# praateekmahajan/moving-mnist-vae

Hardware: AMD Instinct MI355X
Metric: frames/sec/GPU VAE train step, 20×64×64 batch; ELBO vs CPU ref (higher is better)
Workload: dtype bf16; 1 GPU; BASELINE configs[1]: 256 clips x 20 frames x 64x64 per GPU per step (=5120 frames), conv-VAE z=128, Gaussian NLL sigma=0.1 + KL (normal_vae_1_kl_0_mmd), Adam, random-init weights, Bernoulli(0.0521) q=2 labels; parallelism=dp1, rccl_ranks=1, grad_exchange=none, bn=per-rank batch statistics

## Files before the change

include/mmvae.h:

```cpp
#ifndef MMVAE_H_
#define MMVAE_H_

#include <stddef.h>
#include <stdint.h>

#ifdef __cplusplus
extern "C" {
#endif

#if defined(__GNUC__)
#define MMVAE_API __attribute__((visibility("default")))
#else
#define MMVAE_API
#endif

#define MMVAE_OK 0
#define MMVAE_ERR_ARG (-1)
#define MMVAE_ERR_HIP (-2)
#define MMVAE_ERR_WORKSPACE (-3)
#define MMVAE_ERR_UNSUPPORTED (-4)

#define MMVAE_F32 0
#define MMVAE_BF16 1
#define MMVAE_FP8 2
// ... 23 lines not shown
                             void* workspace, size_t workspace_bytes, float* mu, float* logvar, int training, void* stream);
MMVAE_API int mmvae_encoder_bwd(mmvae_net* net, int N, const float* d_mu, const float* d_logvar, const float* params, float* grads,
                      void* workspace, size_t workspace_bytes, void* stream);
MMVAE_API int mmvae_decoder_fwd(mmvae_net* net, int N, const float* encoding, const float* params, float* bn_f32, int64_t* bn_i64,
                      void* workspace, size_t workspace_bytes, float* recon, int training, void* stream);
MMVAE_API int mmvae_decoder_bwd(mmvae_net* net, int N, const float* d_recon, const float* params, float* grads, void* workspace,
                      size_t workspace_bytes, float* d_encoding , void* stream);
MMVAE_API int mmvae_decoder_bwd_gauss(mmvae_net* net, int N, const float* target, float sigma, float coef, const float* gscale, const float* params,
                            float* grads, void* workspace, size_t workspace_bytes, float* d_enc, void* stream);

MMVAE_API int mmvae_net_defer_join(mmvae_net* net, int enable);
MMVAE_API int mmvae_net_join(mmvae_net* net, void* stream);
MMVAE_API void* mmvae_net_fork(mmvae_net* net, void* stream);
MMVAE_API void* mmvae_net_side_stream(mmvae_net* net);
MMVAE_API int mmvae_net_set_join_grad(mmvae_net* net, int enable);
MMVAE_API int mmvae_net_describe_routes(mmvae_net* net, int N, char* buf, int cap);

typedef int (*mmvae_allreduce_fn)(float* buf, int64_t n, void* stream, void* user);
MMVAE_API int mmvae_net_set_sync_bn(mmvae_net* net, mmvae_allreduce_fn fn, void* user, int world);

typedef struct mmvae_comm mmvae_comm;
#define MMVAE_COMM_ID_BYTES 128
MMVAE_API int mmvae_comm_unique_id(void* id_host );
MMVAE_API int mmvae_comm_init(mmvae_comm** out, int world, int rank, const void* id_host);
MMVAE_API int mmvae_comm_allreduce(mmvae_comm* comm, float* buf, int64_t n, void* stream);
MMVAE_API int mmvae_comm_destroy(mmvae_comm* comm);
MMVAE_API int mmvae_net_set_sync_bn_comm(mmvae_net* net, mmvae_comm* comm);
MMVAE_API int mmvae_net_set_sync_bn_comm2(mmvae_net* net, mmvae_comm* comm_main, mmvae_comm* comm_side);

MMVAE_API int mmvae_rsample_fwd(const float* mu, const float* logvar, const float* eps, float* enc, int64_t n, void* stream);
// ... 118 lines not shown
                       void* scratch, void* stream);
MMVAE_API int mmvae_conv2d_wgrad_pair(int dtype, const void* x, const void* dy, const void* dy_shortcut, float* dweight, float* dweight_sc, int N,
                            int H, int W, int Cin, int Cout, const float* pro_scale, const float* pro_shift, int pro_relu, void* scratch,
                            void* stream);
#define MMVAE_BN_SCRATCH_BYTES (16u << 20)
MMVAE_API int mmvae_batchnorm_fwd(int dtype, const void* y, int64_t npix, int C, const float* gamma, const float* beta, float* running_mean,
                        float* running_var, int64_t* nbt, float momentum, float eps, int relu, void* out, float* save_mean, float* save_istd,
                        void* scratch, void* stream);
MMVAE_API int mmvae_batchnorm_bwd(int dtype, const void* dout, const void* y, const void* out, int64_t npix, int C, const float* gamma,
                        const float* save_mean, const float* save_istd, void* dy, float* dgamma, float* dbeta, void* scratch, void* stream);
#define MMVAE_STEM_SCRATCH_BYTES 12800u
MMVAE_API int mmvae_stem_fwd(int dtype, const void* x, const float* weight, void* y, int N, int S, float* stats, void* scratch, void* stream);
MMVAE_API int mmvae_stem_bwd(int dtype, const void* g, const void* y0, const void* x, const float* weight, const float* gamma,
                   const float* bn_scale, const float* bn_shift, const float* save_mean, const float* save_istd, float* dweight,
                   float* dgamma, float* dbeta, int N, int S, void* scratch, void* stream);
MMVAE_API int mmvae_convT_bwd_fused(int dtype, const void* x, const void* dy, const float* weight, float* dweight, void* dx, int N, int H, int W,
                          int Cin, int Cout, int k, int stride, int pad, const float* pro_scale, const float* pro_shift, int pro_relu,
                          const void* x2, const float* w2, float* dw2, void* scratch, void* wscratch, void* stream);
MMVAE_API int mmvae_tail_join_fwd(int dtype, const void* y2, const float* s2, const float* b2, const void* ys, const float* ss, const float* bs,
                        const float* weight, const float* bias, float* r_raw, float* stats, int N, int H, int W, void* stream);
MMVAE_API int mmvae_tail_join_fwd_stream(int dtype, const void* y2, const float* s2, const float* b2, const void* ys, const float* ss, const float* bs,
                               const float* weight, const float* bias, float* r_raw, float* stats, int N, int H, int W, void* stream);
MMVAE_API int mmvae_tail_join_bwd_reduce(int dtype, const float* d_raw, const float* weight, int out_planes, const void* y2, const float* s2,
                               const float* b2, const void* ys, const float* ss, const float* bs, float* partials, float* wpartials,
                               int N, int H, int W, void* stream);
MMVAE_API int mmvae_tail_join_bwd_apply(int dtype, const float* d_raw, const float* weight, int out_planes, const void* y2, const float* s2,
                              const float* b2, const void* ys, const float* ss, const float* bs, const float* A2, const float* B2,
                              const float* C2, const float* As, const float* Bs, const float* Cs, void* dy2, void* dys, int N, int H, int W,
                              void* stream);
MMVAE_API int mmvae_upblock_bwd_fused(const float* d_raw, const float* tail_weight, const void* y2, const float* s2, const float* b2,
// ... 40 lines not shown
```

moving-mnist-vae_amd/_lib.py:

```python
from __future__ import annotations

import ctypes
import os
from ctypes import POINTER, c_char_p, c_double, c_float, c_int, c_int32, c_int64, c_size_t, c_uint64, c_void_p

import torch

_HERE = os.path.dirname(os.path.abspath(__file__))
LIB_PATH = os.environ.get("MMVAE_LIB_PATH") or os.path.join(_HERE, "libmmvae_hip.so")
_lib = None
ABI_VERSION = 3
SUM_PARTIALS = 1025
BN_SCRATCH_BYTES = 16 << 20
STEM_SCRATCH_BYTES = 12800

P = c_void_p

PROTOTYPES = {
    "mmvae_abi_version": (c_int, []),
    "mmvae_last_error": (c_char_p, []),
    "mmvae_net_create": (c_int, [POINTER(c_void_p), c_int, c_int, c_int, c_int, c_int, c_int]),
    "mmvae_net_create_ex": (c_int, [POINTER(c_void_p), c_int, c_int, c_int, c_int, c_int, c_int, c_int]),
    "mmvae_net_destroy": (None, [P]),
    "mmvae_net_sizes": (c_int, [P, POINTER(c_int64), POINTER(c_int64), POINTER(c_int32), POINTER(c_int64), POINTER(c_int32)]),
    "mmvae_net_num_entries": (c_int, [P]),
    "mmvae_net_entry": (c_int, [P, c_int, c_char_p, c_int, POINTER(c_int32), POINTER(c_int32), POINTER(c_int32), POINTER(c_int64)]),
    "mmvae_net_workspace_bytes": (c_size_t, [P, c_int]),
    "mmvae_encoder_fwd": (c_int, [P, c_int, P, P, P, P, P, c_size_t, P, P, c_int, P]),
    "mmvae_net_stage_labels": (c_int, [P, c_int, P, c_int, c_float, c_float, P, P, c_size_t, P]),
    "mmvae_encoder_fwd_staged": (c_int, [P, c_int, P, P, P, P, P, c_size_t, P, P, c_int, P]),
    "mmvae_encoder_bwd": (c_int, [P, c_int, P, P, P, P, P, c_size_t, P]),
    "mmvae_decoder_fwd": (c_int, [P, c_int, P, P, P, P, P, c_size_t, P, c_int, P]),
    "mmvae_decoder_bwd": (c_int, [P, c_int, P, P, P, P, c_size_t, P, P]),
    "mmvae_decoder_bwd_gauss": (c_int, [P, c_int, P, c_float, c_float, P, P, P, P, c_size_t, P, P]),
    "mmvae_net_defer_join": (c_int, [P, c_int]),
    "mmvae_net_join": (c_int, [P, P]),
    "mmvae_net_fork": (P, [P, P]),
    "mmvae_net_side_stream": (P, [P]),
    "mmvae_net_set_join_grad": (c_int, [P, c_int]),
    "mmvae_net_describe_routes": (c_int, [P, c_int, c_char_p, c_int]),
    "mmvae_net_set_sync_bn": (c_int, [P, P, P, c_int]),
    "mmvae_rsample_fwd": (c_int, [P, P, P, P, c_int64, P]),
    "mmvae_rsample_bwd": (c_int, [P, P, P, P, P, c_int64, P]),
    "mmvae_kl_fwd": (c_int, [P, P, c_int64, P, P]),
    "mmvae_kl_fwd_ex": (c_int, [P, P, c_int64, P, P, P]),
    "mmvae_kl_bwd": (c_int, [P, P, c_float, P, P, P, c_int64, P]),
    "mmvae_gauss_nll_fwd": (c_int, [P, P, c_int64, c_float, P, P]),
    "mmvae_gauss_nll_fwd_ex": (c_int, [P, P, c_int64, c_float, P, P, P]),
    "mmvae_gauss_nll_bwd": (c_int, [P, P, c_int64, c_float, c_float, P, P, P]),
    "mmvae_ce_fwd": (c_int, [P, P, P, c_int, c_int, c_int, P, P]),
    "mmvae_ce_fwd_ex": (c_int, [P, P, P, c_int, c_int, c_int, P, P, P]),
    "mmvae_ce_bwd": (c_int, [P, P, P, c_int, c_int, c_int, c_float, P, P, P]),
    "mmvae_mmd_fwd": (c_int, [P, P, c_int, c_int, P, P, P]),
    "mmvae_mmd_fwd_ex": (c_int, [P, P, c_int, c_int, P, P, P, P]),
# ... 32 lines not shown
    "mmvae_conv2d_dgrad_ex": (c_int, [c_int, c_int, P, P, P, c_int, c_int, c_int, c_int, c_int, c_int, c_int, c_int, c_int, P, P, c_int, P, P]),
    "mmvae_conv2d_wgrad": (c_int, [c_int, c_int, P, P, P, c_int, c_int, c_int, c_int, c_int, c_int, c_int, c_int, P, P, c_int, P, P]),
    "mmvae_conv2d_wgrad_pair": (c_int, [c_int, P, P, P, P, P, c_int, c_int, c_int, c_int, c_int, P, P, c_int, P, P]),
    "mmvae_rbf_kernel": (c_int, [P, P, c_int, c_int, c_int, P, P]),
    "mmvae_comm_unique_id": (c_int, [P]),
    "mmvae_comm_init": (c_int, [POINTER(c_void_p), c_int, c_int, P]),
    "mmvae_comm_allreduce": (c_int, [P, P, c_int64, P]),
    "mmvae_comm_destroy": (c_int, [P]),
    "mmvae_net_set_sync_bn_comm": (c_int, [P, P]),
    "mmvae_net_set_sync_bn_comm2": (c_int, [P, P, P]),
    "mmvae_convT_bwd_fused": (c_int, [c_int, P, P, P, P, P, c_int, c_int, c_int, c_int, c_int, c_int, c_int, c_int, P, P, c_int, P, P, P, P, P, P]),
    "mmvae_batchnorm_fwd": (c_int, [c_int, P, c_int64, c_int, P, P, P, P, P, c_float, c_float, c_int, P, P, P, P, P]),
    "mmvae_batchnorm_bwd": (c_int, [c_int, P, P, P, c_int64, c_int, P, P, P, P, P, P, P, P]),
    "mmvae_stem_fwd": (c_int, [c_int, P, P, P, c_int, c_int, P, P, P]),
    "mmvae_stem_bwd": (c_int, [c_int, P, P, P, P, P, P, P, P, P, P, P, P, c_int, c_int, P, P]),
    "mmvae_tail_join_fwd": (c_int, [c_int, P, P, P, P, P, P, P, P, P, P, c_int, c_int, c_int, P]),
    "mmvae_tail_join_fwd_stream": (c_int, [c_int, P, P, P, P, P, P, P, P, P, P, c_int, c_int, c_int, P]),
    "mmvae_tail_join_bwd_reduce": (c_int, [c_int, P, P, c_int, P, P, P, P, P, P, P, P, c_int, c_int, c_int, P]),
    "mmvae_tail_join_bwd_apply": (c_int, [c_int, P, P, c_int, P, P, P, P, P, P, P, P, P, P, P, P, P, P, c_int, c_int, c_int, P]),
    "mmvae_upblock_bwd_fused": (c_int, [P] * 27 + [c_int, P, P]),
    "mmvae_join_conv1x1_fwd": (c_int, [P, P, P, P, P, P, P, c_int, P, P, P, c_int64, P, P]),
    "mmvae_conv1x1_bwd_fused": (c_int, [P] * 13 + [c_int64, P, P]),
    "mmvae_upblock_tail_fwd": (c_int, [P] * 16 + [c_int, P, P]),
    "mmvae_upblock_tail_fwd_store": (c_int, [P] * 18 + [c_int, P, P]),
    "mmvae_convT4_stats": (c_int, [c_int, P, P, P, P, P, c_int, c_int, P, P]),
    "mmvae_pixelcnn_create": (c_int, [POINTER(c_void_p), c_int, c_int, c_int, c_int, c_int]),
    "mmvae_pixelcnn_destroy": (None, [P]),
    "mmvae_pixelcnn_num_params": (c_int64, [P]),
    "mmvae_pixelcnn_workspace_bytes": (c_size_t, [P, c_int, c_int]),
    "mmvae_pixelcnn_fwd": (c_int, [P, c_int, c_int, P, P, P, c_size_t, P, P]),
# ... 82 lines not shown
```

moving-mnist-vae_amd/csrc/capi.cpp:

```cpp
#include <cstring>
#include <new>

#include "../../include/mmvae.h"
#include "conv_ops.hpp"
#include "pixel_net.hpp"
#include "quantiser_fit.hpp"
#include "resample.hpp"
#include "vae_net.hpp"

namespace mmvae { const char* last_error(); }
using namespace mmvae;

struct mmvae_net { Net* net; };
struct mmvae_comm { Comm* c; };

static inline hipStream_t stream_of(void* s) { return static_cast<hipStream_t>(s); }

extern "C" {

int mmvae_abi_version(void) { return MMVAE_ABI_VERSION; }
const char* mmvae_last_error(void) { return last_error(); }

int mmvae_net_create(mmvae_net** out, int in_channels, int z, int out_channels, int image_size, int need_logvar, int dtype) {
  return mmvae_net_create_ex(out, in_channels, z, out_channels, image_size, need_logvar, dtype, 1);
// ... 89 lines not shown
  return MMVAE_OK;
}
int mmvae_net_join(mmvae_net* n, void* stream) {
  if (!n) { set_error("net_join: bad argument"); return MMVAE_ERR_ARG; }
  return n->net->join(stream_of(stream));
}

void* mmvae_net_fork(mmvae_net* n, void* stream) {
  if (!n) return stream;
  return reinterpret_cast<void*>(n->net->fork(stream_of(stream)));
}

int mmvae_net_set_join_grad(mmvae_net* n, int enable) {
  if (!n) { set_error("net_set_join_grad: bad argument"); return MMVAE_ERR_ARG; }
  n->net->set_join_grad(enable != 0);
  return MMVAE_OK;
}

int mmvae_net_describe_routes(mmvae_net* n, int N, char* buf, int cap) {
  if (!n || N <= 0 || cap < 0 || (!buf && cap > 0)) { set_error("net_describe_routes: bad argument"); return MMVAE_ERR_ARG; }
  std::string text;
  const int rc = n->net->describe_routes(N, text);
  if (rc < 0) return rc;
  if (cap > 0) { std::strncpy(buf, text.c_str(), cap - 1); buf[cap - 1] = 0; }
  return (int)text.size() + 1;
}

void* mmvae_net_side_stream(mmvae_net* n) { return n ? reinterpret_cast<void*>(n->net->side()) : nullptr; }

int mmvae_net_set_sync_bn(mmvae_net* n, mmvae_allreduce_fn fn, void* user, int world) {
// ... 446 lines not shown
                   void* scratch, void* st) {
  if (!scratch || N < 1) { set_error("stem_bwd: bad arguments"); return MMVAE_ERR_ARG; }
  if (!stem_bwd_fusable(Sz)) { set_error("stem_bwd: image size %d unsupported (64, 32, 16)", Sz); return MMVAE_ERR_UNSUPPORTED; }
  const int H1 = (Sz + 4 - 5) / 2 + 1;
  double* R = static_cast<double*>(scratch);
  float* gram = reinterpret_cast<float*>(R + 1024);
  const long gram_floats = 1024L * stem_bwd_part_floats();
  float* part = gram + gram_floats;
  const long part_floats = (long)(MMVAE_BN_SCRATCH_BYTES - 1024 * 8) / 4 - gram_floats;
  int rc = launch_stem_gram(dt, x, gram, gram_floats, R, N, Sz, H1, H1, stream_of(st));
  if (rc < 0) return rc;
  const int np = launch_stem_bwd(dt, g, y0, x, bn_scale, bn_shift, part, part_floats, N, Sz, H1, H1, stream_of(st));
  if (np < 0) return np;
  return launch_stem_bwd_finalize(part, np, R, w, nullptr, (double)N * H1 * H1, gamma, save_mean, save_istd, dgamma, dbeta, dw, stream_of(st));
}
int mmvae_tail_join_fwd(int dt, const void* y2, const float* s2, const float* b2, const void* ys, const float* ss, const float* bs,
                        const float* w, const float* bias, float* r_raw, float* stats, int N, int H, int W, void* st) {
  return launch_tail_join_fwd(dt, BnSide{y2, {s2, b2}}, BnSide{ys, {ss, bs}}, w, bias, r_raw, stats, N, H, W, stream_of(st));
}
int mmvae_tail_join_fwd_stream(int dt, const void* y2, const float* s2, const float* b2, const void* ys, const float* ss, const float* bs,
                               const float* w, const float* bias, float* r_raw, float* stats, int N, int H, int W, void* st) {
  return launch_tail_fwd_stream(dt, BnSide{y2, {s2, b2}}, BnSide{ys, {ss, bs}}, w, bias, r_raw, stats, N, H, W, stream_of(st));
}
int mmvae_tail_join_bwd_reduce(int dt, const float* d_raw, const float* w, int oc, const void* y2, const float* s2, const float* b2,
                               const void* ys, const float* ss, const float* bs, float* partials, float* wpartials, int N, int H, int W,
                               void* st) {
  return launch_tail_join_bwd_reduce(dt, d_raw, w, BnSide{y2, {s2, b2}}, BnSide{ys, {ss, bs}}, partials, oc, N, H, W, stream_of(st), wpartials);
}
int mmvae_tail_join_bwd_apply(int dt, const float* d_raw, const float* w, int oc, const void* y2, const float* s2, const float* b2,
                              const void* ys, const float* ss, const float* bs, const float* A2, const float* B2, const float* C2,
// ... 94 lines not shown
```

moving-mnist-vae_amd/csrc/conv_fstream.hip:

```cpp
#include <hip/hip_runtime.h>

#include <stdlib.h>
#include <string.h>

#include "kernels.hpp"
#include "tile_common.hpp"

namespace mmvae {

struct Conv3StreamArgs {
  const void* x; const void* w; const void* wsc; void* y; void* ysc;
  const float* pro_scale; const float* pro_shift; int pro_relu;
  float* stats; float* stats_sc;
  const void* ym; const float* ms; const float* mb;
  int N, Ho, Hi;
  int HS, nunits;
};

template <int S, bool SC, bool PRO, bool BS = false>
__global__ __launch_bounds__(256, 2) void conv3_stream_kernel(Conv3StreamArgs a) {
  static_assert(!BS || (S == 1 && !SC && !PRO), "backward sums: the stride-1 data gradient");
  constexpr int KS = 3, PAD = 1, WO = 16, WI = S * WO, CB = 64;
  constexpr int WL = WI + 2;
  constexpr int ROWB = WL * CB;
  constexpr int NSLOT = KS + S;
  constexpr int WAVE_LDS = NSLOT * ROWB;
  constexpr int RV = S * WI * CB / 1024;
  constexpr int NPRIME = (KS - S + S - 1) / S;
  extern __shared__ __attribute__((aligned(16))) char smem[];
  const int t = threadIdx.x, lane = t & 63, wv = __builtin_amdgcn_readfirstlane(t >> 6), gq = lane >> 4, r = lane & 15;
  char* ring = smem + 2048 + wv * WAVE_LDS;
  for (int s = 0; s < NSLOT; ++s) {
    if (lane < 4) *reinterpret_cast<Vec16*>(ring + s * ROWB + lane * 16) = Vec16{{0, 0, 0, 0}};
    else if (lane < 8) *reinterpret_cast<Vec16*>(ring + s * ROWB + (WL - 1) * CB + (lane - 4) * 16) = Vec16{{0, 0, 0, 0}};
  }
  Vec16 wA[KS * KS][2], wS[2];
#pragma unroll
  for (int m = 0; m < 2; ++m) {
    const int c = 8 * (r >> 2) + 4 * m + (r & 3);
#pragma unroll
    for (int tap = 0; tap < KS * KS; ++tap)
      wA[tap][m] = *reinterpret_cast<const Vec16*>(reinterpret_cast<const char*>(a.w) + ((c * KS * KS + tap) * 32 + 8 * gq) * 2);
    wS[m] = SC ? *reinterpret_cast<const Vec16*>(reinterpret_cast<const char*>(a.wsc) + (c * 32 + 8 * gq) * 2) : Vec16{{0, 0, 0, 0}};
  }
  float psc[8], psh[8];
  if (PRO) {
    const int c = (lane & 3) * 8;
#pragma unroll
    for (int j = 0; j < 8; ++j) { psc[j] = a.pro_scale[c + j]; psh[j] = a.pro_shift[c + j]; }
  }
  const float lo = a.pro_relu ? 0.f : -__builtin_inff();
  float bms[8], bmb[8];
  if (BS) {
#pragma unroll
    for (int j = 0; j < 8; ++j) { bms[j] = a.ms[8 * gq + j]; bmb[j] = a.mb[8 * gq + j]; }
  }
  Vec16 yv = Vec16{{0, 0, 0, 0}};
  float st[SC ? 4 : 2][8];
#pragma unroll
  for (int q = 0; q < (SC ? 4 : 2); ++q)
#pragma unroll
    for (int j = 0; j < 8; ++j) st[q][j] = 0.f;

  const bf16_t* __restrict__ X = reinterpret_cast<const bf16_t*>(a.x);
  const int nblk = gridDim.x;
  int u_first, u_step, u_end;
  if ((nblk & 7) == 0) {
    const int per = (a.nunits + 7) >> 3;
    const int lo_u = (blockIdx.x & 7) * per;
    u_first = lo_u + (blockIdx.x >> 3) * 4 + wv; u_step = (nblk >> 3) * 4; u_end = min(a.nunits, lo_u + per);
  } else { u_first = blockIdx.x * 4 + wv; u_step = nblk * 4; u_end = a.nunits; }
  const int nstrips = a.Ho / a.HS;
  const int nq = a.HS + NPRIME;

  Vec16 xv[RV];
  auto issue = [&](int u, int q) {
    const int n = u / nstrips, oh0 = (u - n * nstrips) * a.HS;
    const int top = S * (oh0 + q - NPRIME) + 1;
#pragma unroll
    for (int k = 0; k < RV; ++k) {
      const int byte = (lane + 64 * k) * 16;
      const int rr = byte / (WI * CB), off = byte - rr * (WI * CB);
      const int row = top - S + 1 + rr;
      xv[k] = Vec16{{0, 0, 0, 0}};
      if (row >= 0 && row < a.Hi) xv[k] = *reinterpret_cast<const Vec16*>(reinterpret_cast<const char*>(X) + (((long)n * a.Hi + row) * WI) * CB + off);
    }
    if (BS && q >= NPRIME)
      yv = *reinterpret_cast<const Vec16*>(reinterpret_cast<const char*>(a.ym) + ((((long)n * a.Ho + oh0 + q - NPRIME) * WO + r) * 32 + 8 * gq) * 2);
  };
  auto commit = [&](int u, int q) {
    const int n = u / nstrips, oh0 = (u - n * nstrips) * a.HS;
    const int top = S * (oh0 + q - NPRIME) + 1;
#pragma unroll
    for (int k = 0; k < RV; ++k) {
      const int byte = (lane + 64 * k) * 16;
      const int rr = byte / (WI * CB), off = byte - rr * (WI * CB);
      const int row = top - S + 1 + rr;
      Vec16 v = xv[k];
      if (PRO && row >= 0 && row < a.Hi) {
        float f[8];
        Elem<bf16_t>::unpack(v, f);
#pragma unroll
        for (int j = 0; j < 8; ++j) f[j] = fmaxf(f[j] * psc[j] + psh[j], lo);
        v = Elem<bf16_t>::pack(f);
      }
      *reinterpret_cast<Vec16*>(ring + ((row + 4 * NSLOT) % NSLOT) * ROWB + CB + off) = v;
    }
    (void)n;
  };

  int u = u_first, q = 0;
  if (u < u_end) issue(u, 0);
  while (u < u_end) {
    commit(u, q);
    const Vec16 ycur = yv;
    int un = u, qn = q + 1;
    if (qn == nq) { un = u + u_step; qn = 0; }
    if (un < u_end) issue(un, qn);
    __builtin_amdgcn_sched_barrier(0);
    if (q >= NPRIME) {
      const int n = u / nstrips, oh = (u - n * nstrips) * a.HS + q - NPRIME;
// ... 49 lines not shown
      if (r == 0) sb[wv * 128 + qq * 32 + 8 * gq + j] = v;
    }
  __syncthreads();
  if (t < (SC ? 128 : 64)) {
    const float v = (sb[t] + sb[128 + t]) + (sb[256 + t] + sb[384 + t]);
    float* dst = t < 64 ? a.stats : a.stats_sc;
    if (dst) dst[(long)blockIdx.x * 64 + (t & 63)] = v;
  }
}

bool conv3_stream_ok(int dt, int Cin, int Cout, int k, int s, int p, int Hin, int Win) {
  return dt == DT_BF16 && Cin == 32 && Cout == 32 && k == 3 && p == 1 && (s == 1 || s == 2) && Hin == Win && Win == 16 * s;
}

int launch_conv3_stream(int dt, int stride, const void* x, const void* w, const void* wsc, void* y, void* ysc, const float* pro_scale,
                        const float* pro_shift, int pro_relu, float* stats, float* stats_sc, int N, int Ho, hipStream_t s) {
  if (dt != DT_BF16 || (stride != 1 && stride != 2) || (wsc && stride != 2) || ((wsc != nullptr) != (ysc != nullptr))) {
    set_error("conv3_stream: bf16, stride 1 or 2, shortcut only with stride 2"); return MMVAE_ERR_UNSUPPORTED;
  }
  Conv3StreamArgs a; memset(&a, 0, sizeof(a));
  a.x = x; a.w = w; a.wsc = wsc; a.y = y; a.ysc = ysc; a.pro_scale = pro_scale; a.pro_shift = pro_shift; a.pro_relu = pro_relu;
  a.stats = stats; a.stats_sc = stats_sc; a.N = N; a.Ho = Ho; a.Hi = stride * Ho;
  a.HS = Ho % 8 == 0 ? 8 : Ho;
  a.nunits = N * (Ho / a.HS);
  int gx = stride == 1 ? 768 : 512;
  while (gx > 8 && (long)gx * 4 > a.nunits) gx -= 8;
  const bool pro = pro_scale != nullptr;
  const size_t lds = 2048 + 4 * (size_t)((3 + stride) * (stride * 16 + 2) * 64);
#define MMVAE_C3(S_, SC_, P_) hipLaunchKernelGGL((conv3_stream_kernel<S_, SC_, P_>), dim3(gx), dim3(256), lds, s, a)
  if (stride == 2) { if (wsc) { if (pro) MMVAE_C3(2, true, true); else MMVAE_C3(2, true, false); } else { if (pro) MMVAE_C3(2, false, true); else MMVAE_C3(2, false, false); } }
  else { if (pro) MMVAE_C3(1, false, true); else MMVAE_C3(1, false, false); }
#undef MMVAE_C3
  note_launch_bytes((double)N * 32 * 2.0 * ((double)a.Hi * a.Hi + (double)Ho * Ho * (wsc ? 2 : 1)));
  const int rc = check_launch("conv3_stream");
  return rc ? rc : gx;
}

int launch_conv3_stream_bwd(int dt, const void* dy, const void* w_flipped, void* dx, const void* ym, const float* ms, const float* mb, float* sums,
                            int N, int H, hipStream_t s) {
  if (dt != DT_BF16 || H != 16 || !ym || !ms || !mb || !sums) { set_error("conv3_stream_bwd: bf16, 16x16 maps, mask operand and sums required"); return MMVAE_ERR_UNSUPPORTED; }
  Conv3StreamArgs a; memset(&a, 0, sizeof(a));
  a.x = dy; a.w = w_flipped; a.y = dx; a.stats = sums; a.ym = ym; a.ms = ms; a.mb = mb; a.N = N; a.Ho = H; a.Hi = H;
  a.HS = 8; a.nunits = N * (H / a.HS);
  int gx = 768;
  while (gx > 8 && (long)gx * 4 > a.nunits) gx -= 8;
  const size_t lds = 2048 + 4 * (size_t)(4 * 18 * 64);
  hipLaunchKernelGGL((conv3_stream_kernel<1, false, false, true>), dim3(gx), dim3(256), lds, s, a);
  note_launch_bytes((double)N * 32 * 2.0 * 3.0 * H * H);
// ... 584 lines not shown
```

moving-mnist-vae_amd/csrc/kernels.hpp:

```cpp
#pragma once
#include "common.hpp"

namespace mmvae {

enum DType : int { DT_F32 = 0, DT_BF16 = 1 };
inline size_t dtype_size(int dt) { return dt == DT_F32 ? 4 : 2; }

struct Affine { const float* scale = nullptr; const float* shift = nullptr; };
struct BnCoef { const float* A = nullptr; const float* B = nullptr; const float* C = nullptr; };
struct BnSide { const void* y = nullptr; Affine fwd; BnCoef bwd; };

struct Tap { int dh, dw; };
constexpr int kMaxTaps = 25;
constexpr int kMaxPhases = 4;
struct Phase { int ph, pw, Hq, Wq, ntaps, tap0; long w_off;  };
struct GatherArgs {
  const void* x; const void* w; void* y;
  const float* pro_scale; const float* pro_shift; int pro_relu;
  const float* bias;
  float* stats;
  int accumulate;
  int N, Hi, Wi, Cin, Ho, Wo, Cout;
  int SI, SO;
  int nphase; Phase phases[kMaxPhases]; Tap taps[kMaxTaps];
// ... 132 lines not shown
  int cols_valid, K_valid;
  int fp8;
  int frag;
};
int launch_pack(int dt, const PackArgs& a, hipStream_t s);
void pack_batch_begin();
int pack_batch_flush(int dt, hipStream_t s);

int launch_stem_im2col(int dt, const void* x, void* col, int N, int H, int W, int Ho, int Wo, hipStream_t s);

bool stem_bwd_fusable(int S);
bool conv3_stream_ok(int dt, int Cin, int Cout, int k, int s, int p, int Hin, int Win);
int launch_conv3_stream_bwd(int dt, const void* dy, const void* w_flipped, void* dx, const void* ym, const float* ms, const float* mb, float* sums,
                            int N, int H, hipStream_t s);
int launch_conv3_stream(int dt, int stride, const void* x, const void* w, const void* wsc, void* y, void* ysc, const float* pro_scale,
                        const float* pro_shift, int pro_relu, float* stats, float* stats_sc, int N, int Ho, hipStream_t s);
bool convT4_stream_ok(int dt, int Cin, int Cout, int k, int s, int p, int Hin, int Win);
int launch_convT4_stream(int dt, const void* x, const void* w_up, void* y, const float* pro_scale, const float* pro_shift, int pro_relu, float* stats,
                         int N, int Hin, hipStream_t s, int f8out = 0);
bool tail_fwd_stream_ok(int dt, int OC, int H, int W);
int launch_tail_fwd_stream(int dt, const BnSide& y2, const BnSide& ys, const float* w, const float* bias, float* r_raw, float* stats, int N, int H,
                           int W, hipStream_t s, int f8in = 0);
bool up5_tail_fwd_ok(int dt, int OC, int C, int Cin, int Hin, int Hout);
int launch_up5_tail_fwd(const BnSide& y1, const void* w2_up, const BnSide& xin, const void* wu_up, Affine bn2, Affine bns, const float* w,
                        const float* bias, float* r_raw, float* stats, int N, hipStream_t s, void* y2 = nullptr, void* ys = nullptr);
bool stem_fwd_stream_ok(int dt, int S);
int launch_stem_fwd_stream(int dt, const void* x, const float* w, void* y, float* stats, int N, int S, hipStream_t s);
int stem_bwd_part_floats();
int launch_stem_gram(int dt, const void* x, float* scratch, long scratch_cap_floats, double* R, int N, int S, int Ho, int Wo, hipStream_t s);
int launch_stem_bwd(int dt, const void* g, const void* y0, const void* x, const float* ms, const float* mb, float* partials,
                    long partials_cap_floats, int N, int S, int Ho, int Wo, hipStream_t s);
// ... 135 lines not shown
```

moving-mnist-vae_amd/csrc/vae_net.cpp:

```cpp
#include "vae_net.hpp"

#include <algorithm>
#include <cmath>
#include <cstdlib>
#include <cstring>

#include "conv_ops.hpp"

namespace mmvae {

#define MM_TRY(expr)            \
  do {                          \
    int rc__ = (expr);          \
    if (rc__ < 0) return rc__;  \
  } while (0)

static inline long align_up(long v, long a) { return (v + a - 1) / a * a; }
static inline int down_size(int H, int k, int s, int p) { return conv_down_size(H, k, s, p); }

void Net::add_entry(const std::string& name, std::initializer_list<int> shape, int kind, long off) {
  Entry e; e.name = name; e.ndim = (int)shape.size(); e.kind = kind; e.offset = off;
  int i = 0; for (int d : shape) e.shape[i++] = d;
  for (; i < 4; ++i) e.shape[i] = 1;
  entries.push_back(e);
// ... 583 lines not shown
    np = launch_gather_gemm(dt(), dt(), a, s);
  }
  MM_TRY(np);
  MM_TRY(bn_fwd(ps, bn0, np, (double)N * H1 * W1, s));
  const void* xin = base + P.y0;
  const float* xs = ps.rows(bn0).scale;
  const float* xb = ps.rows(bn0).shift;
  if (cfg.blocks > 1) MM_TRY(fill_consts(ps, s));
  for (size_t i = 0; i < enc.size(); ++i) {
    Block& B = enc[i];
    const double cnt = (double)N * B.Hout * B.Wout;
    const BnRows r1 = ps.rows(B.b1);
    const BnSide s2 = ps.rows(B.b2).side(base + B.y2), sc = ps.shortcut(B, xin);
    const bool stream1 = B.r.fwd_c1_cs_stream, stream2 = B.r.fwd_c2_stream, fork = !B.identity && !stream1;
    if (stream1) {
      np = launch_conv3_stream(dt(), 2, xin, ps.packed(B.c1.packD), ps.packed(B.cs.packD), base + B.y1,
                               base + B.ys, xs, xb, 1, stats, stats ? stats + kPartialFloats : nullptr, N, B.Hout, s);
      MM_TRY(np);
      MM_TRY(bn_fwd(ps, B.bs, np, cnt, s, kPartialFloats, B.cs.wscale));
      MM_TRY(bn_fwd(ps, B.b1, np, cnt, s, 0, B.c1.wscale));
    } else if (!B.identity) {
      if (fork) MM_TRY(side_fork(s));
      hipStream_t ss = fork ? wgrad_stream(s) : s;
      np = run_down(ps, B.cs, xin, B.Hin, B.Win, base + B.ys, B.Hout, B.Wout, xs, xb, 1, stats ? stats + kPartialFloats : nullptr, 0, dt(), ss);
      MM_TRY(np);
      MM_TRY(bn_fwd(ps, B.bs, np, cnt, ss, kPartialFloats, B.cs.wscale));
    }
    if (!stream1) {
      np = run_down(ps, B.c1, xin, B.Hin, B.Win, base + B.y1, B.Hout, B.Wout, xs, xb, 1, stats, 0, dt(), s);
      MM_TRY(np);
      MM_TRY(bn_fwd(ps, B.b1, np, cnt, s, 0, B.c1.wscale));
    }
// ... 397 lines not shown
```

moving-mnist-vae_amd/csrc/vae_net.hpp:

```cpp
#pragma once
#include <string>
#include <vector>

#include "comm.hpp"
#include "conv_ops.hpp"
#include "kernels.hpp"

namespace mmvae {

struct NetCfg { int in_ch, z, out_ch, S, need_logvar, dtype, blocks, fp8; };

enum EntryKind : int { EK_PARAM = 0, EK_BN_F32 = 1, EK_BN_I64 = 2 };
struct Entry { std::string name; int ndim; int shape[4]; int kind; long offset; };

struct ConvW { long off; int D0, D1, k, s, p; long packD, packU; int Hl = 0;  bool tr = false;  bool fp8 = false; float wscale = 1.f;
               bool fragD = false, fragU = false;  };
struct Bn {
  long g_off, b_off, rm_off, rv_off; int nbt_idx; int C; long ws;
  enum Row { MEAN, ISTD, SCALE, SHIFT, COEF_A, COEF_B, COEF_C, kRows };
  long row_floats() const { return (C + 3L) / 4 * 4; }
  long row(Row r) const { return ws + r * row_floats(); }
  long scratch_floats() const { return kRows * row_floats(); }
};
struct BnRows {
// ... 132 lines not shown
               const ConvW* w2 = nullptr, const void* x2 = nullptr);
  int run_up(const Pass& ps, const ConvW& w, const void* S, int Hs, int Ws, void* L, int Hl, int Wl,
             const float* pro_s, const float* pro_b, int relu, float* stats, int accumulate, hipStream_t s,
             const ConvW* w2 = nullptr, const void* x2 = nullptr);
  int run_wgrad(const Pass& ps, const ConvW& w, const void* P, int Hs, int Ws, const float* proP_s, const float* proP_b,
                const void* G, int Hl, int Wl, const float* proG_s, const float* proG_b, hipStream_t s);
  int reduce_wgrad_parts(const Pass& ps, const ConvW& w, const float* parts, int nparts, int ntaps, hipStream_t s);
  bool defer_join_ = false;
  int (*ar_fn_)(float*, long long, void*, void*) = nullptr; void* ar_user_ = nullptr; int ar_world_ = 1;
  Comm* comm_ = nullptr; Comm* comm_side_ = nullptr;
  int sync_rows(const Pass& ps, const float* partials, int nparts, int width, hipStream_t s, float** out, int row_stride = 0);
 public:
  void set_defer_join(bool v) { defer_join_ = v; }
  bool join_grad_ = true;
  void set_join_grad(bool v) { join_grad_ = v; plan_.N = -1; }
  typedef int (*AllReduceFn)(float* buf, long long n, void* stream, void* user);
  void set_sync_bn(AllReduceFn fn, void* user, int world) { ar_fn_ = fn; ar_user_ = user; ar_world_ = fn ? world : 1; comm_ = comm_side_ = nullptr; }
  void set_sync_bn_comm(Comm* c, Comm* side = nullptr) { comm_ = c; comm_side_ = c ? side : nullptr; ar_fn_ = nullptr; ar_user_ = nullptr; ar_world_ = c ? comm_world(c) : 1; }
  bool sync_bn_on() const { return ar_fn_ != nullptr || comm_ != nullptr; }
  int join(hipStream_t s) { return side_join(s); }
  hipStream_t side() const { return side_state_ == 1 ? side_ : nullptr; }
  hipStream_t fork(hipStream_t s) { return side_fork(s) == MMVAE_OK ? wgrad_stream(s) : s; }
 private:
  int bn_fwd(const Pass& ps, const Bn& bn, int nparts, double count, hipStream_t s, long part_off = 0, float in_scale = 1.f);
  int fold_bn_eval(const Pass& ps, int which, hipStream_t s);
  long l1c2_flip = 0; bool eval_folded_ = false;
  bool store8 = false;
  int fill_consts(const Pass& ps, hipStream_t s);
  int bn_backward_coefs(const Pass& ps, const Bn& bn, int nparts, int ny, int which, double count, hipStream_t s, float* dbias_conv = nullptr);
  BnBwdFinalizeArgs bwd_finalize_args(const Pass& ps, const Bn& bn, const float* partials, int nparts, int ny, int which, double count) const;
// ... 8 lines not shown
```

Before: 867,300 frames/s.

## Recompute stem conv output inside encoder layer1 kernel from the raw image

In training with a 64x64 input, the encoder layer1 stride-2 conv kernel now reads the raw bf16 image. It recomputes the stem's 5x5 conv output on the fly with MFMA, then applies BN+ReLU before the 3x3 conv and shortcut. This avoids reading the 32-channel stem activation back from global memory. The cost is extra LDS for an image patch ring, redundant stem arithmetic per tile, and a second rounding path that must match the stored stem output used in backward.

Result: no change. 870,000 frames/s, median of 5 (+0.3%).

```diff
diff --git a/include/mmvae.h b/include/mmvae.h
--- a/include/mmvae.h
+++ b/include/mmvae.h
@@ -61,6 +61,7 @@
 MMVAE_API void* mmvae_net_fork(mmvae_net* net, void* stream);
 MMVAE_API void* mmvae_net_side_stream(mmvae_net* net);
 MMVAE_API int mmvae_net_set_join_grad(mmvae_net* net, int enable);
+MMVAE_API int mmvae_net_set_stem_recompute(mmvae_net* net, int enable);
 MMVAE_API int mmvae_net_describe_routes(mmvae_net* net, int N, char* buf, int cap);
 
 typedef int (*mmvae_allreduce_fn)(float* buf, int64_t n, void* stream, void* user);
@@ -209,6 +210,8 @@
 MMVAE_API int mmvae_stem_bwd(int dtype, const void* g, const void* y0, const void* x, const float* weight, const float* gamma,
                    const float* bn_scale, const float* bn_shift, const float* save_mean, const float* save_istd, float* dweight,
                    float* dgamma, float* dbeta, int N, int S, void* scratch, void* stream);
+MMVAE_API int mmvae_stem_block1_fwd(int dtype, const void* x, const float* weight, const float* bn_scale, const float* bn_shift, const float* w1,
+                          const float* ws, void* y1, void* ys, float* stats1, float* stats_s, int N, int S, void* scratch, void* stream);
 MMVAE_API int mmvae_convT_bwd_fused(int dtype, const void* x, const void* dy, const float* weight, float* dweight, void* dx, int N, int H, int W,
                           int Cin, int Cout, int k, int stride, int pad, const float* pro_scale, const float* pro_shift, int pro_relu,
                           const void* x2, const float* w2, float* dw2, void* scratch, void* wscratch, void* stream);
diff --git a/moving-mnist-vae_amd/_lib.py b/moving-mnist-vae_amd/_lib.py
--- a/moving-mnist-vae_amd/_lib.py
+++ b/moving-mnist-vae_amd/_lib.py
@@ -38,6 +38,7 @@
     "mmvae_net_fork": (P, [P, P]),
     "mmvae_net_side_stream": (P, [P]),
     "mmvae_net_set_join_grad": (c_int, [P, c_int]),
+    "mmvae_net_set_stem_recompute": (c_int, [P, c_int]),
     "mmvae_net_describe_routes": (c_int, [P, c_int, c_char_p, c_int]),
     "mmvae_net_set_sync_bn": (c_int, [P, P, P, c_int]),
     "mmvae_rsample_fwd": (c_int, [P, P, P, P, c_int64, P]),
@@ -100,6 +101,7 @@
     "mmvae_batchnorm_bwd": (c_int, [c_int, P, P, P, c_int64, c_int, P, P, P, P, P, P, P, P]),
     "mmvae_stem_fwd": (c_int, [c_int, P, P, P, c_int, c_int, P, P, P]),
     "mmvae_stem_bwd": (c_int, [c_int, P, P, P, P, P, P, P, P, P, P, P, P, c_int, c_int, P, P]),
+    "mmvae_stem_block1_fwd": (c_int, [c_int] + [P] * 10 + [c_int, c_int, P, P]),
     "mmvae_tail_join_fwd": (c_int, [c_int, P, P, P, P, P, P, P, P, P, P, c_int, c_int, c_int, P]),
     "mmvae_tail_join_fwd_stream": (c_int, [c_int, P, P, P, P, P, P, P, P, P, P, c_int, c_int, c_int, P]),
     "mmvae_tail_join_bwd_reduce": (c_int, [c_int, P, P, c_int, P, P, P, P, P, P, P, P, c_int, c_int, c_int, P]),
diff --git a/moving-mnist-vae_amd/csrc/capi.cpp b/moving-mnist-vae_amd/csrc/capi.cpp
--- a/moving-mnist-vae_amd/csrc/capi.cpp
+++ b/moving-mnist-vae_amd/csrc/capi.cpp
@@ -127,6 +127,12 @@
 int mmvae_net_set_join_grad(mmvae_net* n, int enable) {
   if (!n) { set_error("net_set_join_grad: bad argument"); return MMVAE_ERR_ARG; }
   n->net->set_join_grad(enable != 0);
+  return MMVAE_OK;
+}
+
+int mmvae_net_set_stem_recompute(mmvae_net* n, int enable) {
+  if (!n) { set_error("net_set_stem_recompute: bad argument"); return MMVAE_ERR_ARG; }
+  n->net->set_stem_recompute(enable != 0);
   return MMVAE_OK;
 }
 
@@ -603,6 +609,16 @@
   if (np < 0) return np;
   return launch_stem_bwd_finalize(part, np, R, w, nullptr, (double)N * H1 * H1, gamma, save_mean, save_istd, dgamma, dbeta, dw, stream_of(st));
 }
+int mmvae_stem_block1_fwd(int dt, const void* x, const float* w, const float* bn_scale, const float* bn_shift, const float* w1, const float* ws,
+                          void* y1, void* ys, float* stats1, float* stats_s, int N, int Sz, void* scratch, void* st) {
+  if (!scratch || !x || !w || !bn_scale || !bn_shift || !w1 || !ws || !y1 || !ys || N < 1) { set_error("stem_block1_fwd: bad arguments"); return MMVAE_ERR_ARG; }
+  if (dt != DT_BF16 || Sz != 64 || !stem_fwd_stream_ok(dt, Sz)) { set_error("stem_block1_fwd: bf16 and 64 x 64 images only"); return MMVAE_ERR_UNSUPPORTED; }
+  char* p1 = static_cast<char*>(scratch);
+  char* ps = p1 + 32 * 32 * 9 * 2;
+  int rc = op_pack_down(dt, geom_for(0, 32, 32, 3, 2, 1), w1, p1, stream_of(st)); if (rc < 0) return rc;
+  rc = op_pack_down(dt, geom_for(0, 32, 32, 1, 2, 0), ws, ps, stream_of(st)); if (rc < 0) return rc;
+  return launch_conv3_stream(dt, 2, nullptr, p1, ps, y1, ys, bn_scale, bn_shift, 1, stats1, stats_s, N, 16, stream_of(st), x, w);
+}
 int mmvae_tail_join_fwd(int dt, const void* y2, const float* s2, const float* b2, const void* ys, const float* ss, const float* bs,
                         const float* w, const float* bias, float* r_raw, float* stats, int N, int H, int W, void* st) {
   return launch_tail_join_fwd(dt, BnSide{y2, {s2, b2}}, BnSide{ys, {ss, bs}}, w, bias, r_raw, stats, N, H, W, stream_of(st));
diff --git a/moving-mnist-vae_amd/csrc/conv_fstream.hip b/moving-mnist-vae_amd/csrc/conv_fstream.hip
--- a/moving-mnist-vae_amd/csrc/conv_fstream.hip
+++ b/moving-mnist-vae_amd/csrc/conv_fstream.hip
@@ -13,18 +13,22 @@
   const float* pro_scale; const float* pro_shift; int pro_relu;
   float* stats; float* stats_sc;
   const void* ym; const float* ms; const float* mb;
+  const void* img; const float* w0;
   int N, Ho, Hi;
   int HS, nunits;
 };
 
-template <int S, bool SC, bool PRO, bool BS = false>
+constexpr int kImgPw = 72, kImgSlots = 8;
+
+template <int S, bool SC, bool PRO, bool BS = false, bool IMG = false>
 __global__ __launch_bounds__(256, 2) void conv3_stream_kernel(Conv3StreamArgs a) {
   static_assert(!BS || (S == 1 && !SC && !PRO), "backward sums: the stride-1 data gradient");
+  static_assert(!IMG || (S == 2 && PRO && !BS), "input rows from the image: the stride-2 conv behind the stem's BatchNorm + ReLU");
   constexpr int KS = 3, PAD = 1, WO = 16, WI = S * WO, CB = 64;
   constexpr int WL = WI + 2;
   constexpr int ROWB = WL * CB;
   constexpr int NSLOT = KS + S;
-  constexpr int WAVE_LDS = NSLOT * ROWB;
+  constexpr int WAVE_LDS = NSLOT * ROWB + (IMG ? kImgSlots * kImgPw * 4 : 0);
   constexpr int RV = S * WI * CB / 1024;
   constexpr int NPRIME = (KS - S + S - 1) / S;
   extern __shared__ __attribute__((aligned(16))) char smem[];
@@ -43,9 +47,26 @@
       wA[tap][m] = *reinterpret_cast<const Vec16*>(reinterpret_cast<const char*>(a.w) + ((c * KS * KS + tap) * 32 + 8 * gq) * 2);
     wS[m] = SC ? *reinterpret_cast<const Vec16*>(reinterpret_cast<const char*>(a.wsc) + (c * 32 + 8 * gq) * 2) : Vec16{{0, 0, 0, 0}};
   }
+  float* const patch = reinterpret_cast<float*>(ring + NSLOT * ROWB);
+  Vec16 wA0[2];
+  int toff[8];
+  const bool tap_in = gq < 3;
+  if constexpr (IMG) {
+    for (int i = lane; i < kImgSlots * kImgPw; i += 64) patch[i] = 0.f;
+#pragma unroll
+    for (int m = 0; m < 2; ++m) {
+      const int c = 8 * (r >> 2) + 4 * m + (r & 3);
+      float f[8];
+#pragma unroll
+      for (int j = 0; j < 8; ++j) { const int tap = 8 * gq + j; f[j] = tap < 25 ? a.w0[c * 25 + tap] : 0.f; }
+      wA0[m] = Elem<bf16_t>::pack(f);
+    }
+#pragma unroll
+    for (int j = 0; j < 8; ++j) { const int tap = 8 * gq + j; toff[j] = tap < 25 ? (tap / 5) * kImgPw + tap % 5 + 2 * r + 2 : 0; }
+  }
   float psc[8], psh[8];
   if (PRO) {
-    const int c = (lane & 3) * 8;
+    const int c = (IMG ? gq : (lane & 3)) * 8;
 #pragma unroll
     for (int j = 0; j < 8; ++j) { psc[j] = a.pro_scale[c + j]; psh[j] = a.pro_shift[c + j]; }
   }
@@ -73,38 +94,86 @@
   const int nstrips = a.Ho / a.HS;
   const int nq = a.HS + NPRIME;
 
-  Vec16 xv[RV];
+  Vec16 xv[IMG ? 1 : RV];
+  const int irow = lane >> 3, icol = (lane & 7) * 8;
   auto issue = [&](int u, int q) {
     const int n = u / nstrips, oh0 = (u - n * nstrips) * a.HS;
     const int top = S * (oh0 + q - NPRIME) + 1;
-#pragma unroll
-    for (int k = 0; k < RV; ++k) {
-      const int byte = (lane + 64 * k) * 16;
-      const int rr = byte / (WI * CB), off = byte - rr * (WI * CB);
-      const int row = top - S + 1 + rr;
-      xv[k] = Vec16{{0, 0, 0, 0}};
-      if (row >= 0 && row < a.Hi) xv[k] = *reinterpret_cast<const Vec16*>(reinterpret_cast<const char*>(X) + (((long)n * a.Hi + row) * WI) * CB + off);
-    }
-    if (BS && q >= NPRIME)
-      yv = *reinterpret_cast<const Vec16*>(reinterpret_cast<const char*>(a.ym) + ((((long)n * a.Ho + oh0 + q - NPRIME) * WO + r) * 32 + 8 * gq) * 2);
+    if constexpr (IMG) {
+      const int row = 2 * (top - 1) - 2 + irow;
+      xv[0] = Vec16{{0, 0, 0, 0}};
+      if (irow < 7 && (q == 0 || irow >= 3) && row >= 0 && row < 2 * a.Hi)
+        xv[0] = *reinterpret_cast<const Vec16*>(reinterpret_cast<const bf16_t*>(a.img) + (((long)n * 2 * a.Hi + row) * (2 * WI) + icol));
+    } else {
+#pragma unroll
+      for (int k = 0; k < RV; ++k) {
+        const int byte = (lane + 64 * k) * 16;
+        const int rr = byte / (WI * CB), off = byte - rr * (WI * CB);
+        const int row = top - S + 1 + rr;
+        xv[k] = Vec16{{0, 0, 0, 0}};
+        if (row >= 0 && row < a.Hi) xv[k] = *reinterpret_cast<const Vec16*>(reinterpret_cast<const char*>(X) + (((long)n * a.Hi + row) * WI) * CB + off);
+      }
+      if (BS && q >= NPRIME)
+        yv = *reinterpret_cast<const Vec16*>(reinterpret_cast<const char*>(a.ym) + ((((long)n * a.Ho + oh0 + q - NPRIME) * WO + r) * 32 + 8 * gq) * 2);
+    }
   };
   auto commit = [&](int u, int q) {
     const int n = u / nstrips, oh0 = (u - n * nstrips) * a.HS;
     const int top = S * (oh0 + q - NPRIME) + 1;
-#pragma unroll
-    for (int k = 0; k < RV; ++k) {
-      const int byte = (lane + 64 * k) * 16;
-      const int rr = byte / (WI * CB), off = byte - rr * (WI * CB);
-      const int row = top - S + 1 + rr;
-      Vec16 v = xv[k];
-      if (PRO && row >= 0 && row < a.Hi) {
+    if constexpr (IMG) {
+      const int rb = 2 * (top - 1) - 2;
+      if (irow < 7 && (q == 0 || irow >= 3)) {
         float f[8];
-        Elem<bf16_t>::unpack(v, f);
-#pragma unroll
-        for (int j = 0; j < 8; ++j) f[j] = fmaxf(f[j] * psc[j] + psh[j], lo);
-        v = Elem<bf16_t>::pack(f);
-      }
-      *reinterpret_cast<Vec16*>(ring + ((row + 4 * NSLOT) % NSLOT) * ROWB + CB + off) = v;
+        Elem<bf16_t>::unpack(xv[0], f);
+        float* d = patch + ((rb + irow) & (kImgSlots - 1)) * kImgPw + 4 + icol;
+        *reinterpret_cast<float4*>(d) = make_float4(f[0], f[1], f[2], f[3]);
+        *reinterpret_cast<float4*>(d + 4) = make_float4(f[4], f[5], f[6], f[7]);
+      }
+#pragma unroll
+      for (int e = 0; e < 2; ++e) {
+        const int row = top - 1 + e;
+        char* dst = ring + ((row + 4 * NSLOT) % NSLOT) * ROWB + CB + r * CB + gq * 16;
+        if (row >= 0 && row < a.Hi) {
+          const int s0 = ((rb + 2 * e) & (kImgSlots - 1)) * kImgPw;
+          int to[8];
+#pragma unroll
+          for (int j = 0; j < 8; ++j) { const unsigned v = toff[j] + s0; to[j] = (int)min(v, v - kImgSlots * kImgPw); }
+#pragma unroll
+          for (int pt = 0; pt < 2; ++pt) {
+            float f[8];
+#pragma unroll
+            for (int j = 0; j < 8; ++j) { const float g = patch[to[j] + 32 * pt]; f[j] = (j == 0 || tap_in) ? g : 0.f; }
+            const Vec16 bf = Elem<bf16_t>::pack(f);
+            const f32x4 z = (f32x4){0, 0, 0, 0};
+            const f32x4 d0 = mma_bf16(wA0[0], bf, z), d1 = mma_bf16(wA0[1], bf, z);
+            const float v[8] = {d0[0], d0[1], d0[2], d0[3], d1[0], d1[1], d1[2], d1[3]};
+            float y[8];
+            Elem<bf16_t>::unpack(Elem<bf16_t>::pack(v), y);
+#pragma unroll
+            for (int j = 0; j < 8; ++j) y[j] = fmaxf(y[j] * psc[j] + psh[j], lo);
+            *reinterpret_cast<Vec16*>(dst + pt * 16 * CB) = Elem<bf16_t>::pack(y);
+          }
+        } else {
+          *reinterpret_cast<Vec16*>(dst) = Vec16{{0, 0, 0, 0}};
+          *reinterpret_cast<Vec16*>(dst + 16 * CB) = Vec16{{0, 0, 0, 0}};
+        }
+      }
+    } else {
+#pragma unroll
+      for (int k = 0; k < RV; ++k) {
+        const int byte = (lane + 64 * k) * 16;
+        const int rr = byte / (WI * CB), off = byte - rr * (WI * CB);
+        const int row = top - S + 1 + rr;
+        Vec16 v = xv[k];
+        if (PRO && row >= 0 && row < a.Hi) {
+          float f[8];
+          Elem<bf16_t>::unpack(v, f);
+#pragma unroll
+          for (int j = 0; j < 8; ++j) f[j] = fmaxf(f[j] * psc[j] + psh[j], lo);
+          v = Elem<bf16_t>::pack(f);
+        }
+        *reinterpret_cast<Vec16*>(ring + ((row + 4 * NSLOT) % NSLOT) * ROWB + CB + off) = v;
+      }
     }
     (void)n;
   };
@@ -184,11 +253,17 @@
 }
 
 int launch_conv3_stream(int dt, int stride, const void* x, const void* w, const void* wsc, void* y, void* ysc, const float* pro_scale,
-                        const float* pro_shift, int pro_relu, float* stats, float* stats_sc, int N, int Ho, hipStream_t s) {
+                        const float* pro_shift, int pro_relu, float* stats, float* stats_sc, int N, int Ho, hipStream_t s, const void* img,
+                        const float* w0) {
   if (dt != DT_BF16 || (stride != 1 && stride != 2) || (wsc && stride != 2) || ((wsc != nullptr) != (ysc != nullptr))) {
     set_error("conv3_stream: bf16, stride 1 or 2, shortcut only with stride 2"); return MMVAE_ERR_UNSUPPORTED;
   }
+  if (img && (x || !w0 || stride != 2 || !wsc || !pro_scale || !pro_shift || Ho != 16)) {
+    set_error("conv3_stream: the input is recomputed from the image only for encoder.layer1 behind the stem (stride 2, shortcut, prologue, 16 x 16 output)");
+    return MMVAE_ERR_UNSUPPORTED;
+  }
   Conv3StreamArgs a; memset(&a, 0, sizeof(a));
+  a.img = img; a.w0 = w0;
   a.x = x; a.w = w; a.wsc = wsc; a.y = y; a.ysc = ysc; a.pro_scale = pro_scale; a.pro_shift = pro_shift; a.pro_relu = pro_relu;
   a.stats = stats; a.stats_sc = stats_sc; a.N = N; a.Ho = Ho; a.Hi = stride * Ho;
   a.HS = Ho % 8 == 0 ? 8 : Ho;
@@ -196,12 +271,14 @@
   int gx = stride == 1 ? 768 : 512;
   while (gx > 8 && (long)gx * 4 > a.nunits) gx -= 8;
   const bool pro = pro_scale != nullptr;
-  const size_t lds = 2048 + 4 * (size_t)((3 + stride) * (stride * 16 + 2) * 64);
+  const size_t lds = 2048 + 4 * (size_t)((3 + stride) * (stride * 16 + 2) * 64 + (img ? kImgSlots * kImgPw * 4 : 0));
 #define MMVAE_C3(S_, SC_, P_) hipLaunchKernelGGL((conv3_stream_kernel<S_, SC_, P_>), dim3(gx), dim3(256), lds, s, a)
-  if (stride == 2) { if (wsc) { if (pro) MMVAE_C3(2, true, true); else MMVAE_C3(2, true, false); } else { if (pro) MMVAE_C3(2, false, true); else MMVAE_C3(2, false, false); } }
+  if (img) hipLaunchKernelGGL((conv3_stream_kernel<2, true, true, false, true>), dim3(gx), dim3(256), lds, s, a);
+  else if (stride == 2) { if (wsc) { if (pro) MMVAE_C3(2, true, true); else MMVAE_C3(2, true, false); } else { if (pro) MMVAE_C3(2, false, true); else MMVAE_C3(2, false, false); } }
   else { if (pro) MMVAE_C3(1, false, true); else MMVAE_C3(1, false, false); }
 #undef MMVAE_C3
-  note_launch_bytes((double)N * 32 * 2.0 * ((double)a.Hi * a.Hi + (double)Ho * Ho * (wsc ? 2 : 1)));
+  note_launch_bytes(img ? (double)N * 2.0 * (4.0 * a.Hi * a.Hi + 32.0 * Ho * Ho * 2)
+                        : (double)N * 32 * 2.0 * ((double)a.Hi * a.Hi + (double)Ho * Ho * (wsc ? 2 : 1)));
   const int rc = check_launch("conv3_stream");
   return rc ? rc : gx;
 }
diff --git a/moving-mnist-vae_amd/csrc/kernels.hpp b/moving-mnist-vae_amd/csrc/kernels.hpp
--- a/moving-mnist-vae_amd/csrc/kernels.hpp
+++ b/moving-mnist-vae_amd/csrc/kernels.hpp
@@ -170,7 +170,8 @@
 int launch_conv3_stream_bwd(int dt, const void* dy, const void* w_flipped, void* dx, const void* ym, const float* ms, const float* mb, float* sums,
                             int N, int H, hipStream_t s);
 int launch_conv3_stream(int dt, int stride, const void* x, const void* w, const void* wsc, void* y, void* ysc, const float* pro_scale,
-                        const float* pro_shift, int pro_relu, float* stats, float* stats_sc, int N, int Ho, hipStream_t s);
+                        const float* pro_shift, int pro_relu, float* stats, float* stats_sc, int N, int Ho, hipStream_t s, const void* img = nullptr,
+                        const float* w0 = nullptr);
 bool convT4_stream_ok(int dt, int Cin, int Cout, int k, int s, int p, int Hin, int Win);
 int launch_convT4_stream(int dt, const void* x, const void* w_up, void* y, const float* pro_scale, const float* pro_shift, int pro_relu, float* stats,
                          int N, int Hin, hipStream_t s, int f8out = 0);
diff --git a/moving-mnist-vae_amd/csrc/vae_net.cpp b/moving-mnist-vae_amd/csrc/vae_net.cpp
--- a/moving-mnist-vae_amd/csrc/vae_net.cpp
+++ b/moving-mnist-vae_amd/csrc/vae_net.cpp
@@ -621,8 +621,10 @@
     const BnSide s2 = ps.rows(B.b2).side(base + B.y2), sc = ps.shortcut(B, xin);
     const bool stream1 = B.r.fwd_c1_cs_stream, stream2 = B.r.fwd_c2_stream, fork = !B.identity && !stream1;
     if (stream1) {
-      np = launch_conv3_stream(dt(), 2, xin, ps.packed(B.c1.packD), ps.packed(B.cs.packD), base + B.y1,
-                               base + B.ys, xs, xb, 1, stats, stats ? stats + kPartialFloats : nullptr, N, B.Hout, s);
+      const bool from_img = i == 0 && training && P.route.stem_fwd_stream && stem_recompute_ && cfg.S == 64;
+      np = launch_conv3_stream(dt(), 2, from_img ? nullptr : xin, ps.packed(B.c1.packD), ps.packed(B.cs.packD), base + B.y1,
+                               base + B.ys, xs, xb, 1, stats, stats ? stats + kPartialFloats : nullptr, N, B.Hout, s,
+                               from_img ? base + P.x_t : nullptr, from_img ? params + stem.off : nullptr);
       MM_TRY(np);
       MM_TRY(bn_fwd(ps, B.bs, np, cnt, s, kPartialFloats, B.cs.wscale));
       MM_TRY(bn_fwd(ps, B.b1, np, cnt, s, 0, B.c1.wscale));
diff --git a/moving-mnist-vae_amd/csrc/vae_net.hpp b/moving-mnist-vae_amd/csrc/vae_net.hpp
--- a/moving-mnist-vae_amd/csrc/vae_net.hpp
+++ b/moving-mnist-vae_amd/csrc/vae_net.hpp
@@ -170,6 +170,8 @@
   void set_defer_join(bool v) { defer_join_ = v; }
   bool join_grad_ = true;
   void set_join_grad(bool v) { join_grad_ = v; plan_.N = -1; }
+  bool stem_recompute_ = true;
+  void set_stem_recompute(bool v) { stem_recompute_ = v; plan_.N = -1; }
   typedef int (*AllReduceFn)(float* buf, long long n, void* stream, void* user);
   void set_sync_bn(AllReduceFn fn, void* user, int world) { ar_fn_ = fn; ar_user_ = user; ar_world_ = fn ? world : 1; comm_ = comm_side_ = nullptr; }
   void set_sync_bn_comm(Comm* c, Comm* side = nullptr) { comm_ = c; comm_side_ = c ? side : nullptr; ar_fn_ = nullptr; ar_user_ = nullptr; ar_world_ = c ? comm_world(c) : 1; }
```
